# fmfi-compbio/nadavca

Hardware: AMD Instinct MI355X
Metric: reads/sec (align_signal, ~4k-sample reads) (higher is better)
Workload: dtype f64

## Files before the change

### nadavca_amd/csrc/api.hip

```cpp
#include <math.h>
#include <stdarg.h>
#include <stdio.h>
#include <stdlib.h>
#include <string.h>

#include <new>
#include <vector>

#include "nvk_internal.h"

static thread_local char g_err[512] = "";

void nvk_set_error(const char *fmt, ...) {
  va_list ap;
  va_start(ap, fmt);
  vsnprintf(g_err, sizeof g_err, fmt, ap);
  va_end(ap);
}

extern "C" const char *nvk_last_error(void) { return g_err; }

extern "C" int nvk_device_count(void) {
  int n = 0;
  if (hipGetDeviceCount(&n) != hipSuccess) return 0;
// ... 36 lines not shown

int64_t nvk_spill_cap(nvk_ctx *ctx, int which_ws) {
  if (ctx->ws_limit > 0) return ctx->ws_limit;
  const int share = ctx->spill_share > 1 ? ctx->spill_share : 1;
  int64_t cap = ((int64_t)48 << 30) / share;
  size_t free_b = 0, total_b = 0;
  if (hipMemGetInfo(&free_b, &total_b) == hipSuccess)
    cap = (int64_t)((double)(free_b + ctx->ws_bytes[which_ws]) * 0.6 / share);
  const int64_t floor_b = (int64_t)64 << 20;
  return cap > floor_b ? cap : floor_b;
}

TimerScope::TimerScope(nvk_ctx *c, int kid) : ctx(c), id(kid) {
  if (ctx->timing_on) (void)hipEventRecord(ctx->ev0, ctx->stream);
}
TimerScope::~TimerScope() {
  if (ctx->timing_on) {
    (void)hipEventRecord(ctx->ev1, ctx->stream);
    (void)hipEventSynchronize(ctx->ev1);
    float ms = 0.f;
    if (hipEventElapsedTime(&ms, ctx->ev0, ctx->ev1) == hipSuccess) {
      ctx->k_ms[id] += (double)ms;
      ctx->k_launches[id] += 1;
    }
  }
}

extern "C" int nvk_ctx_create(int device, nvk_ctx **out) {
  if (!out) {
    nvk_set_error("nvk_ctx_create: out is NULL");
    return NVK_ERR_INVALID;
  }
  *out = nullptr;
// ... 311 lines not shown
      !anc_off || !out_status) {
    nvk_set_error("negative total or NULL offset/status pointer");
    return NVK_ERR_INVALID;
  }
  NVK_HIP(hipSetDevice(model->ctx->device));
  a = BatchArgs{n_reads, total_signal, total_ref, total_anchors, signal, sig_off, reference, ref_off,
                ctx_before, cb_off, ctx_after, ca_off, anchors, anc_off, bandwidth, mel};
  return NVK_OK;
}

struct PlanHost {
  PlanTotals tot;
  int32_t steps[1];
};

int plan_batch(nvk_model *model, const BatchArgs &a, int mode, PlanTotals &tot, const int **order,
               const int32_t **steps_sorted) {
  nvk_ctx *ctx = model->ctx;
  int64_t n = a.n_reads;
  int64_t rows_total = (mode == PLAN_ALIGN_TRANS) ? 2 * a.total_ref : a.total_ref + n;
  int rc;
  if ((rc = nvk_ws_reserve(ctx, WS_META, (size_t)(n + 1) * sizeof(ReadMeta) + 64))) return rc;
  if ((rc = nvk_ws_reserve(ctx, WS_ROWS, (size_t)(rows_total + 1) * sizeof(RowParam)))) return rc;
  if ((rc = nvk_ws_reserve(ctx, WS_BANDTMP, (size_t)(2 * (a.total_ref + n) + 2) * 8))) return rc;
  if ((rc = nvk_ws_reserve(ctx, WS_MISC, 256))) return rc;
  if ((rc = nvk_ws_reserve(ctx, WS_LANE_F, (size_t)(rows_total + 1) * 48))) return rc;
  if ((rc = nvk_ws_reserve(ctx, WS_LANE_R, (size_t)(rows_total + 1) * 48))) return rc;
  if ((rc = nvk_ws_reserve(ctx, WS_OFFS, (size_t)(rows_total + 1) * sizeof(int32_t)))) return rc;
  if ((rc = nvk_ws_reserve(ctx, WS_STEPS, (size_t)(n + 1) * sizeof(int32_t)))) return rc;
  if ((rc = nvk_grow(&ctx->h_plan, &ctx->h_plan_cap, sizeof(PlanHost) + (size_t)n * sizeof(int32_t), true,
                     "planner results")))
    return rc;
  PlanHost *hp = (PlanHost *)ctx->h_plan;
  PlanTotals *d_tot = nvk_plan_totals(ctx);
  rc = launch_plan(ctx, model->dm, a, mode, (ReadMeta *)ctx->ws[WS_META],
                   (RowParam *)ctx->ws[WS_ROWS], (unsigned long long *)ctx->ws[WS_BANDTMP], d_tot,
                   ctx->ws[WS_LANE_F], ctx->ws[WS_LANE_R], (int32_t *)ctx->ws[WS_OFFS]);
  if (rc) return rc;
  int *ord = nullptr;
  rc = launch_order(ctx, (const ReadMeta *)ctx->ws[WS_META], n, d_tot, &ord, (int32_t *)ctx->ws[WS_STEPS]);
  if (rc) return rc;
  NVK_HIP(hipMemcpyAsync(&hp->tot, d_tot, sizeof(PlanTotals), hipMemcpyDeviceToHost, ctx->stream));
  if (n) NVK_HIP(hipMemcpyAsync(hp->steps, ctx->ws[WS_STEPS], (size_t)n * sizeof(int32_t), hipMemcpyDeviceToHost,
                                ctx->stream));
  NVK_HIP(hipStreamSynchronize(ctx->stream));
  tot = hp->tot;
  *order = ord;
  *steps_sorted = hp->steps;
  ctx->last_cells = (int64_t)tot.cells;
  ctx->last_steps = (int64_t)tot.steps;
  return NVK_OK;
}

}

extern "C" int nvk_expected_signal_batch_dev(nvk_model *model, int64_t n_reads, int64_t total_ref,
                                             const int32_t *reference, const int64_t *ref_off,
                                             const int32_t *ctx_before, const int64_t *cb_off,
                                             const int32_t *ctx_after, const int64_t *ca_off,
                                             double *out) {
  int rc = check_common(model, n_reads, 0, 0);
  if (rc) return rc;
  nvk_ctx *ctx = model->ctx;
  NVK_HIP(hipSetDevice(ctx->device));
  rc = launch_expected(ctx, model->dm, n_reads, total_ref, reference, ref_off, ctx_before, cb_off,
// ... 42 lines not shown
    const int32_t *ctx_after, const int64_t *ca_off, const int32_t *anchors,
    const int64_t *anc_off, int bandwidth, int min_event_length, int model_transitions,
    int32_t *out_events, int32_t *out_status) {
  BatchArgs a;
  int rc = dev_batch(model, n_reads, total_signal, total_ref, total_anchors, signal, sig_off, reference, ref_off,
                     ctx_before, cb_off, ctx_after, ca_off, anchors, anc_off, bandwidth, min_event_length,
                     out_status, a);
  if (rc || n_reads == 0) return rc;
  nvk_ctx *ctx = model->ctx;
  PlanTotals tot;
  const char *force = getenv("NADAVCA_ALIGN_KERNEL");
  ctx->last_retries = 0;
  ctx->last_ties = ctx->last_ties_exact = ctx->last_ties_near = ctx->last_ties_ulp = 0;
  const int *order = nullptr;
  const int32_t *steps_sorted = nullptr;
  rc = plan_batch(model, a, model_transitions ? PLAN_ALIGN_TRANS : PLAN_ALIGN_PLAIN, tot, &order, &steps_sorted);
  if (rc) return rc;
  if ((rc = nvk_ws_reserve(ctx, WS_TIES, (size_t)(n_reads + 8) * sizeof(int32_t)))) return rc;
  NVK_HIP(hipMemsetAsync(ctx->ws[WS_TIES], 0, (size_t)(n_reads + 8) * sizeof(int32_t), ctx->stream));
  ctx->ties_n = n_reads;
  ctx->ties_host = nullptr;
  int32_t *d_ties = (int32_t *)ctx->ws[WS_TIES];
  int *d_retry = (int *)(d_ties + n_reads + 4);
  const ReadMeta *metas = (const ReadMeta *)ctx->ws[WS_META];
  const RowParam *rows = (const RowParam *)ctx->ws[WS_ROWS];
  bool exact_all = force && force[0] == '1';
  int32_t tail[5] = {0, 0, 0, 0, 0};
  auto fetch_counts = [&]() -> int {
    int rc2 = launch_count_flags(ctx, d_ties, n_reads, d_ties + n_reads);
    if (rc2) return rc2;
    NVK_HIP(hipMemcpyAsync(tail, d_ties + n_reads, sizeof tail, hipMemcpyDeviceToHost, ctx->stream));
    NVK_HIP(hipStreamSynchronize(ctx->stream));
    return NVK_OK;
  };
  if (!exact_all) {
    rc = launch_align3(ctx, a, model_transitions ? 1 : 0, metas, tot, order, steps_sorted, out_events, out_status,
                       d_retry);
    if (rc) return rc;
    if ((rc = fetch_counts())) return rc;
    ctx->last_retries = tail[4];
    if (tail[4] > 0) {
      rc = launch_align_retry(ctx, a, model_transitions ? 1 : 0, metas, rows, tot, out_events,
                              out_status);
      if (rc) return rc;
      if ((rc = fetch_counts())) return rc;
    }
  } else {
    rc = launch_align(ctx, a, model_transitions ? 1 : 0, metas, rows, tot, out_events, out_status);
    if (rc) return rc;
    if ((rc = fetch_counts())) return rc;
  }
  ctx->last_ties = tail[0];
  ctx->last_ties_exact = tail[1];
  ctx->last_ties_near = tail[2];
  ctx->last_ties_ulp = tail[3];
  return NVK_OK;
}

namespace {
int ell_run(nvk_model *model, const BatchArgs &a, int model_wobbling, double *out_ll, int32_t *out_status,
            const EllHyp &hyp) {
  int rc;
  const int64_t n_reads = a.n_reads, total_ref = a.total_ref;
  nvk_ctx *ctx = model->ctx;
  const int64_t n = n_reads, nrow = total_ref + n;
  if ((rc = nvk_ws_reserve(ctx, WS_META, (size_t)(n + 1) * sizeof(ReadMeta) + 64))) return rc;
  if ((rc = nvk_ws_reserve(ctx, WS_ROWS, (size_t)(total_ref + 1) * sizeof(FusedParam)))) return rc;
  if ((rc = nvk_ws_reserve(ctx, WS_ROWS2, (size_t)(total_ref + 1) * sizeof(FusedParam)))) return rc;
  if ((rc = nvk_ws_reserve(ctx, WS_BP, (size_t)(3 * nrow + 16) * sizeof(int32_t)))) return rc;
  if ((rc = nvk_ws_reserve(ctx, WS_BANDTMP, (size_t)(2 * nrow + 2) * 8))) return rc;
  if ((rc = nvk_ws_reserve(ctx, WS_MISC, 256))) return rc;
  EllPlan pl;
  pl.metas = (ReadMeta *)ctx->ws[WS_META];
  pl.fwd = (FusedParam *)ctx->ws[WS_ROWS];
  pl.rev = (FusedParam *)ctx->ws[WS_ROWS2];
  pl.bs = (int32_t *)ctx->ws[WS_BP];
  pl.be = pl.bs + nrow;
  pl.rowoff = pl.be + nrow;
  PlanTotals *d_tot = nvk_plan_totals(ctx);
  rc = launch_plan_ell(ctx, model->dm, a, model_wobbling ? 1 : 0, pl,
                       (unsigned long long *)ctx->ws[WS_BANDTMP], d_tot);
// ... 135 lines not shown
```

### nadavca_amd/csrc/kernels_align3.hip

```cpp
#include <math.h>

#include <new>
#include <vector>

#include "nvk_internal.h"
#include "xmath.h"
#include "dens.h"
#include "lane3.h"
#include "wave.h"

namespace {

using dens::density;
using dens::density_begin;
using dens::density_end;
using dens::DensHalf;
using dens::ETN;

constexpr int CH = 64;
static_assert(CH == 64, "a refill is one sample per lane");
constexpr int PF = 8;
constexpr int RU = 16;
constexpr int FT = 16;
static_assert(FT % PF == 0 && 32 % FT == 0, "forward trip");
static_assert(32 % PF == 0 && PF % 2 == 0 && 32 % RU == 0 && RU % 2 == 0, "the step count is a multiple of 32 (kernels_plan.hip)");
constexpr int GBIG = 1 << 24;
constexpr int DMAX = 1000;
constexpr int TARGET = 250;
#define HUGE_V 0x1.0p+900
#define MASS_TOL 1e-9
#define TIE_FLAG_REL (1.0 / (double)(1ull << NVK_TIE_BITS))

typedef int v4i_t __attribute__((ext_vector_type(4)));
__device__ __forceinline__ void spill_store2(__amdgpu_buffer_rsrc_t rs, int lane16, int pair, double v_even,
                                             double v_odd) {
  __builtin_amdgcn_raw_buffer_store_b128(__builtin_bit_cast(v4i_t, make_double2(v_even, v_odd)), rs, lane16,
                                         pair * 1024, 0);
}
__device__ __forceinline__ double2 spill_load2(__amdgpu_buffer_rsrc_t rs, int lane16, int pair) {
  return __builtin_bit_cast(double2, __builtin_amdgcn_raw_buffer_load_b128(rs, lane16, pair * 1024, 0));
}

#define STEP_SYNC()                                                              \
  do {                                                                           \
    if (W == 1) WAVE_SYNC();                                                     \
    else asm volatile("s_waitcnt lgkmcnt(0)\n\ts_barrier" ::: "memory");         \
  } while (0)
#define RING_SYNC()                 \
  do {                              \
    if (W == 1) __syncthreads();    \
    else WAVE_SYNC();               \
  } while (0)

struct Align3Args {
  const ReadMeta *metas;
// ... 779 lines not shown
}

bool select_sweeps(int mel, bool pair, int W, int rsh, Align3Kernel k[2]) {
  switch (mel) {
    case 0: return sweeps_of<0>(pair, W, rsh, k);
    case 1: return sweeps_of<1>(pair, W, rsh, k);
    case 2: return sweeps_of<2>(pair, W, rsh, k);
    case 3: return sweeps_of<3>(pair, W, rsh, k);
    case 4: return sweeps_of<4>(pair, W, rsh, k);
    default: return false;
  }
}

}

int launch_align3(nvk_ctx *ctx, const BatchArgs &a, int transitions, const ReadMeta *metas, const PlanTotals &tot,
                  const int *order, const int32_t *steps_sorted, int32_t *out_events, int32_t *out_status,
                  int *d_retry) {
  static_assert(WS_OFFS < (int)(sizeof(ctx->ws) / sizeof(ctx->ws[0])), "workspace table too small");
  if (a.n_reads == 0) return NVK_OK;
  const int mel = a.mel;
  if (mel < 0 || mel > 4) {
    nvk_set_error("min_event_length %d outside the compiled range 0..4", mel);
    return NVK_ERR_UNSUPPORTED;
  }
  const int max_c = tot.max_c < 1 ? 1 : tot.max_c;
  int rc = nvk_ws_reserve(ctx, WS_MISC, 256);
  if (rc) return rc;
  constexpr int N_COUNTERS = 16;
  static_assert(N_COUNTERS % 2 == 0, "a chunk's reverse / forward pair of counters must not straddle a re-zero");
  int *counter = (int *)ctx->ws[WS_MISC];
  int launches = 0;
  NVK_HIP(hipMemsetAsync(d_retry, 0, sizeof(int), ctx->stream));

  constexpr int C_HARD = 24;
  static_assert(ALIGN1_C_CAP + 4 < 8 && C_HARD + 4 < 32, "no kernel for the rescale period these skews need");
  struct Cls { int hi; int W; };
  Cls cls[2];
  int ncls = 0;
  const int64_t n_wide = (int64_t)tot.n_wide;
  const int max_cw = tot.max_cw < 1 ? 1 : tot.max_cw;
  if (a.n_reads - n_wide > 0 || max_c <= ALIGN1_C_CAP)
    cls[ncls++] = Cls{max_c < ALIGN1_C_CAP ? max_c : ALIGN1_C_CAP, 1};
  if (max_c > ALIGN1_C_CAP) cls[ncls++] = Cls{max_cw < C_HARD ? max_cw : C_HARD, ALIGN3_TEAM_W};
  rc = nvk_ws_reserve(ctx, WS_RSTATE, (size_t)a.n_reads * sizeof(int2));
  if (rc) return rc;
  TimerScope ts_align(ctx, NVK_K_ALIGN);
  for (int k = 0; k < ncls; k++) {
    int c = cls[k].hi;
    const int W = cls[k].W, TLk = 64 * W;
    auto lds_need = [&](int cc, int slot_bytes) {
      const int Hc = (cc + mel > 0 ? cc + mel : 1) + (W > 1 ? 1 : 0);
      int SRc = 256;
      while (SRc < 64 * cc + CH) SRc <<= 1;
      return (size_t)ETN * 8 + (size_t)W * SRc * 8 + (size_t)Hc * TLk * slot_bytes + slot_bytes + 16 + 12 * W;
    };
    while (c > 1 && lds_need(c, 20) > 160 * 1024) --c;
    int rsh = transitions ? 4 : 3;
    while ((1 << rsh) <= c + mel) rsh++;
    Align3Kernel kern[2];
    if (!select_sweeps(mel, transitions != 0, W, rsh, kern)) {
// ... 4 lines not shown
    const int H = (c + mel > 0 ? c + mel : 1) + (W > 1 ? 1 : 0);
    int SR = 256;
    while (SR < 64 * c + CH) SR <<= 1;
    const size_t lds = lds_need(c, 20);
    const size_t lds_rev = lds_need(c, 8);
    if (lds > 160 * 1024) return NVK_ERR_UNSUPPORTED;
    int per_cu = (int)((160 * 1024) / lds);
    if (per_cu > 4 * LB / W) per_cu = 4 * LB / W;
    if (per_cu < 1) per_cu = 1;
    int per_cu_rev = (int)((160 * 1024) / lds_rev);
    if (per_cu_rev > 4 * (W > 1 ? LB_REV_TEAM : LB_REV) / W) per_cu_rev = 4 * (W > 1 ? LB_REV_TEAM : LB_REV) / W;
    if (per_cu_rev < 1) per_cu_rev = 1;
    int32_t mxpad = 1;
    for (int64_t q = 0; q < a.n_reads; q++) mxpad = steps_sorted[q] > mxpad ? steps_sorted[q] : mxpad;
    const int64_t bp_stride = (int64_t)((mxpad + 31) / 32 + 1) * TLk;
    const int64_t cap = nvk_spill_cap(ctx, WS_SPILL);

    Align3Args g;
    g.metas = metas;
    g.fwdl = (const Lane3 *)ctx->ws[WS_LANE_F];
    g.revl = (const Lane3 *)ctx->ws[WS_LANE_R];
    g.offs = (const int32_t *)ctx->ws[WS_OFFS];
    g.signal = a.signal;
    g.bp_stride = bp_stride;
    g.order = order;
    g.H = H;
    g.SR = SR;
    g.transitions = transitions;
    g.c_cap = c;
    g.flag_above = (k == ncls - 1) ? 1 : 0;
    g.rstate = (int2 *)ctx->ws[WS_RSTATE];
// ... 30 lines not shown
      rc = nvk_ws_reserve(ctx, WS_STAGE, (size_t)n_chunk * L_stride * 4);
      if (rc) return rc;
      int64_t slots_f = ctx->slots_override > 0 ? ctx->slots_override : (int64_t)ctx->num_cus * per_cu;
      int64_t slots_r = ctx->slots_override > 0 ? ctx->slots_override : (int64_t)ctx->num_cus * per_cu_rev;
      if (slots_f > n_chunk) slots_f = n_chunk;
      if (slots_r > n_chunk) slots_r = n_chunk;
      rc = nvk_ws_reserve(ctx, WS_BP, (size_t)slots_f * bp_stride * 4);
      if (rc) return rc;
      g.spill_v = (double *)ctx->ws[WS_SPILL];
      g.spill_L = (int32_t *)ctx->ws[WS_STAGE];
      g.bp = (uint32_t *)ctx->ws[WS_BP];
      g.spill_stride = spill_stride;
      g.L_stride = L_stride;
      g.n_reads = (int)n_chunk;
      g.read_lo = (int)lo;
      if (launches % N_COUNTERS == 0) NVK_HIP(hipMemsetAsync(counter, 0, N_COUNTERS * sizeof(int), ctx->stream));
      g.counter = counter + launches % N_COUNTERS;
      hipLaunchKernelGGL(kern[0], dim3((unsigned)slots_r), dim3(TLk), lds_rev, ctx->stream, g);
      g.counter = counter + (launches + 1) % N_COUNTERS;
      hipLaunchKernelGGL(kern[1], dim3((unsigned)slots_f), dim3(TLk), lds, ctx->stream, g);
      launches += 2;
      NVK_HIP(hipGetLastError());
      lo = hi;
    }
  }
  ctx->last_spill_bytes = (int64_t)tot.steps * 64 * 16 + (int64_t)tot.steps / 16 * 8 + (int64_t)tot.steps * 8 * 2;
  return NVK_OK;
}
```

### nadavca_amd/csrc/kernels_plan.hip

```cpp
#include <math.h>

#include "nvk_internal.h"
#include "kmer.h"
#include "lane3.h"
#include "wave.h"

namespace {

__device__ __forceinline__ int read_is_bad(const DeviceModel &dm, const BatchArgs &a, int rd, int tid,
                                           int nthreads) {
  const int64_t s0 = a.sig_off[rd], s1 = a.sig_off[rd + 1], r0 = a.ref_off[rd], r1 = a.ref_off[rd + 1];
  const int64_t a0 = a.anc_off[rd], a1 = a.anc_off[rd + 1];
  const int64_t b0 = a.cb_off[rd], b1 = a.cb_off[rd + 1], c0 = a.ca_off[rd], c1 = a.ca_off[rd + 1];
  const int64_t N64 = s1 - s0, R64 = r1 - r0;
  if (s0 < 0 || r0 < 0 || a0 < 0 || b0 < 0 || c0 < 0 || a1 < a0 || b1 < b0 || c1 < c0 ||
      s1 > a.total_signal || r1 > a.total_ref || a1 > a.total_anchors || b1 - b0 > 0x3fffffff ||
      c1 - c0 > 0x3fffffff)
    return 1;
  if (R64 < 1 || N64 < 1 || N64 > 0x3fffffff || R64 > 0x1fffffff) return 1;
  const int R = (int)R64, A = (int)(a1 - a0), nb = (int)(b1 - b0), na = (int)(c1 - c0);
  const int32_t *anc = a.anchors + 2 * a0;
  const int32_t *ref = a.reference + r0, *cb = a.ctx_before + b0, *ca = a.ctx_after + c0;
  int bad = 0;
  for (int j = tid; j < A && !bad; j += nthreads) {
// ... 119 lines not shown
        unsigned long long w = tbe[j];
        v = (w >> 32) ? (int)(unsigned int)(w & 0xffffffffu) - 1 : N;
      } else {
        v = 0x7fffffff;
      }
      v = min(wave_scan_min_dpp(v), carry);
      carry = __builtin_amdgcn_readlane(v, 63);
      if (j <= R) be[j] = v;
    }
  }
  __syncthreads();
}

__device__ __forceinline__ void plan_rows_lds(const DeviceModel &dm, const PlanRead &q, int mode, double log_p_in,
                                              int c_cap, int rd, ReadMeta m, ReadMeta *metas, RowParam *rows,
                                              Lane3 *lane_f, Lane3 *lane_r, int32_t *lane_offs, PlanShared &sh) {
  const int tid = threadIdx.x, lane = tid & 63, wv = tid >> 6;
  const int32_t *ref = q.ref, *cb = q.cb, *ca = q.ca;
  const int N = q.N, R = q.R, T = q.T, nb = q.nb, na = q.na, mel = q.mel;
  const bool trans = (mode == PLAN_ALIGN_TRANS);
  constexpr int VT = PLAN_VT;
  int *sh_x = (int *)sh.pool, *sh_S = sh_x + VT;
  int *sh_bs = sh_S + VT, *sh_be = sh_bs + PLAN_BCAP;
  plan_bands_lds(q.anc, q.A, R, N, q.bw, sh.pool, sh.pool + PLAN_BCAP, sh_bs, sh_be, tid);

  auto rmel = [=](int r) { return (r + 1 < T && !(trans && (r & 1))) ? mel : 0; };
  auto BS = [=](int r) { return sh_bs[trans ? (r + 1) >> 1 : r]; };
  auto BE = [=](int r) { return sh_be[trans ? (r + 1) >> 1 : r]; };
  auto LO = [=](int r) {
    int lo = BS(r);
    if (r > 0) {
// ... 181 lines not shown
    }
    RowParam p, nx;
    p.mean = __shfl_up(o.mean, 1, 64);
    p.ac = __shfl_up(o.ac, 1, 64);
    p.mc = __shfl_up(o.mc, 1, 64);
    p.bs = p.be = p.lo = p.hi = p.mel = p.off = 0;
    nx.mean = nx.ac = nx.mc = 0.0;
    nx.bs = nx.be = nx.lo = nx.hi = nx.mel = nx.off = 0;
    if (have && lane > 0) {
      o.bs = BS(r);
      o.be = BE(r);
      o.lo = LO(r);
      o.hi = HI(r);
      o.off = OFF(r);
      if (!trans && r > 0 && r + 1 < T) plateau |= (p.mean == o.mean) ? 1 : 0;
      rp[r] = o;
      if (records) {
        if (r > 0) {
          p.bs = BS(r - 1);
          p.be = BE(r - 1);
          p.mel = rmel(r - 1);
          p.off = OFF(r - 1);
        }
        if (r < top) {
          nx.bs = BS(r + 1);
          nx.be = BE(r + 1);
          nx.off = OFF(r + 1);
        }
        const int adv_f = (r >= ST) ? o.off - OFF(r - ST) : 0;
        const int adv_b = (r + ST <= top) ? OFF(r + ST) - o.off : 0;
        Lane3 f, b;
// ... 211 lines not shown
    m.cw = cw;
    m.t_min = t_min;
    m.n_steps = t_max - t_min + 1;
    m.pad = rp[T - 1].hi + off_top - t_min + 1;
    m.pad = (m.pad + 31) & ~31;
    m.cells = cells;
    m.rsv = plateau ? 1 : 0;
    if (badband) m.status = NVK_READ_BAD_BAND;
    metas[rd] = m;
  }
}

__global__ __launch_bounds__(PLAN_T, 5) void plan_kernel(DeviceModel dm, BatchArgs a, int mode,
                                                  double log_p_in, int c_cap, ReadMeta *metas,
                                                  RowParam *rows, unsigned long long *bandtmp,
                                                  Lane3 *lane_f, Lane3 *lane_r, int32_t *lane_offs) {
  const int rd = blockIdx.x;
  const int tid = threadIdx.x;
  __shared__ PlanShared sh;
  if (rd >= a.n_reads) return;
  if (tid == 0) {
    sh.cells = 0ull;
    sh.c = 1;
  }
  const int64_t s0 = a.sig_off[rd], r0 = a.ref_off[rd], a0 = a.anc_off[rd];
  const int64_t N64 = a.sig_off[rd + 1] - s0;
  const int64_t R64 = a.ref_off[rd + 1] - r0;
  const int64_t A64 = a.anc_off[rd + 1] - a0;
  PlanRead q;
  q.nb = (int)(a.cb_off[rd + 1] - a.cb_off[rd]);
  q.na = (int)(a.ca_off[rd + 1] - a.ca_off[rd]);
// ... 26 lines not shown
    m.row_off = r0 + rd;
  }
  m.T = q.T;
  m.c = 1;
  m.t_min = 0;
  m.n_steps = 0;

  int bad = read_is_bad(dm, a, rd, tid, PLAN_T);
  bad = __syncthreads_or(bad);
  if (bad) {
    m.status = NVK_READ_BAD_INPUT;
    if (tid == 0) metas[rd] = m;
    return;
  }
  if (q.R + 1 <= PLAN_BCAP && dm.n <= 0x100000000ll)
    plan_rows_lds(dm, q, mode, log_p_in, c_cap, rd, m, metas, rows, lane_f, lane_r, lane_offs, sh);
  else
    plan_rows_global(dm, q, mode, log_p_in, c_cap, rd, m, metas, rows, bandtmp, lane_f, lane_r, lane_offs, sh);
}

__global__ __launch_bounds__(256) void plan_totals_kernel(const ReadMeta *metas, int n, int c_cap, PlanTotals *totals) {
  const int rd = blockIdx.x * 256 + threadIdx.x, lane = threadIdx.x & 63, wv = threadIdx.x >> 6;
  int steps = 0, c = 0, cw = 0, T = 0, wide = 0;
  unsigned long long cells = 0ull, pad = 0ull;
  if (rd < n) {
    const ReadMeta m = metas[rd];
    if (m.status == NVK_READ_OK) {
      steps = max(m.n_steps, 0), c = max(m.c, 0), cw = max(m.cw, 0), T = max(m.T, 0);
      wide = (m.c > c_cap) ? 1 : 0;
      cells = (unsigned long long)m.cells;
      pad = (unsigned long long)m.pad;
// ... 161 lines not shown
  int pos = (int)(g - ref_off[rd]);
  const int32_t *ref = reference + ref_off[rd], *cb = cbs + cb_off[rd], *ca = cas + ca_off[rd];
  const int64_t id = kmer_id_checked(dm, ref, R, cb, nb, ca, na, pos);
  out[g] = id >= 0 ? dm.mean[id] : (double)NAN;
}


constexpr int ORD_B = 64;
constexpr int ORD_N = 2 * ORD_B;
__device__ __forceinline__ int order_bucket(const ReadMeta &m, int max_steps) {
  if (m.status != NVK_READ_OK) return ORD_N - 1;
  long long b = (long long)m.n_steps * ORD_B / ((long long)max_steps + 1);
  const int sb = ORD_B - 1 - (int)(b < 0 ? 0 : (b > ORD_B - 1 ? ORD_B - 1 : b));
  return (m.cw != 0 ? 0 : ORD_B) + sb;
}
__global__ void order_count_kernel(const ReadMeta *metas, int n, const PlanTotals *tot, int *cnt) {
  int rd = blockIdx.x * blockDim.x + threadIdx.x;
  if (rd < n) atomicAdd(&cnt[order_bucket(metas[rd], tot->max_steps)], 1);
}
__global__ void order_scan_kernel(int *cnt) {
  int lane = threadIdx.x;
  const int v0 = cnt[2 * lane], v1 = cnt[2 * lane + 1], s = wave_scan_add(v0 + v1, lane);
  cnt[2 * lane] = s - v0 - v1;
  cnt[2 * lane + 1] = s - v1;
  cnt[ORD_N + 2 * lane] = 0;
  cnt[ORD_N + 2 * lane + 1] = 0;
}
__global__ void order_fill_kernel(const ReadMeta *metas, int n, const PlanTotals *tot, int *cnt, int *order,
                                  int32_t *steps_out) {
  int rd = blockIdx.x * blockDim.x + threadIdx.x;
  if (rd < n) {
    const ReadMeta m = metas[rd];
    int b = order_bucket(m, tot->max_steps);
    const int pos = cnt[b] + atomicAdd(&cnt[ORD_N + b], 1);
    order[pos] = rd;
    if (steps_out) steps_out[pos] = (m.status == NVK_READ_OK) ? m.pad : 0;
  }
}

__global__ void count_flags_kernel(const int32_t *flags, int64_t n, int32_t *out) {
  int64_t g = (int64_t)blockIdx.x * blockDim.x + threadIdx.x;
  const int f = (g < n) ? flags[g] : 0;
  int v = ((f & 7) != 0) ? 1 : 0, v0 = f & 1, v1 = (f >> 1) & 1, v2 = (f >> 2) & 1;
  v = wave_sum(v), v0 = wave_sum(v0), v1 = wave_sum(v1), v2 = wave_sum(v2);
  if ((threadIdx.x & 63) == 0 && v) {
    atomicAdd(out, v);
    if (v0) atomicAdd(out + 1, v0);
    if (v1) atomicAdd(out + 2, v1);
    if (v2) atomicAdd(out + 3, v2);
// ... 21 lines not shown
  int *cnt = ord + n_reads;
  NVK_HIP(hipMemsetAsync(cnt, 0, 2 * ORD_N * sizeof(int), ctx->stream));
  const unsigned blocks = (unsigned)((n_reads + 255) / 256);
  TimerScope ts(ctx, NVK_K_PLAN);
  hipLaunchKernelGGL(order_count_kernel, dim3(blocks), dim3(256), 0, ctx->stream, metas, (int)n_reads, tot_dev, cnt);
  hipLaunchKernelGGL(order_scan_kernel, dim3(1), dim3(64), 0, ctx->stream, cnt);
  hipLaunchKernelGGL(order_fill_kernel, dim3(blocks), dim3(256), 0, ctx->stream, metas, (int)n_reads, tot_dev, cnt, ord,
                     steps_out);
  NVK_HIP(hipGetLastError());
  *order = ord;
  return NVK_OK;
}

int launch_plan(nvk_ctx *ctx, const DeviceModel &dm, const BatchArgs &a, int mode,
                ReadMeta *metas, RowParam *rows, unsigned long long *bandtmp, PlanTotals *totals,
                void *lane_f, void *lane_r, int32_t *lane_offs) {
  NVK_HIP(hipMemsetAsync(totals, 0, sizeof(PlanTotals), ctx->stream));
  if (a.n_reads == 0) return NVK_OK;
  {
    TimerScope ts(ctx, NVK_K_PLAN);
    const double log_p_in = log(0.01);
    hipLaunchKernelGGL(plan_kernel, dim3((unsigned)a.n_reads), dim3(PLAN_T), 0, ctx->stream, dm, a, mode,
                       log_p_in, ALIGN1_C_CAP, metas, rows, bandtmp, (Lane3 *)lane_f, (Lane3 *)lane_r, lane_offs);
    hipLaunchKernelGGL(plan_totals_kernel, dim3((unsigned)((a.n_reads + 255) / 256)), dim3(256), 0, ctx->stream,
                       metas, (int)a.n_reads, ALIGN1_C_CAP, totals);
  }
  NVK_HIP(hipGetLastError());
  return NVK_OK;
}

int launch_plan_ell(nvk_ctx *ctx, const DeviceModel &dm, const BatchArgs &a, int wobbling,
                    const EllPlan &pl, unsigned long long *bandtmp, PlanTotals *totals) {
  NVK_HIP(hipMemsetAsync(totals, 0, sizeof(PlanTotals), ctx->stream));
  if (a.n_reads == 0) return NVK_OK;
  {
    TimerScope ts(ctx, NVK_K_PLAN);
    hipLaunchKernelGGL(plan_ell_kernel, dim3((unsigned)a.n_reads), dim3(64), 0, ctx->stream, dm, a,
                       wobbling, pl, bandtmp, totals);
  }
  NVK_HIP(hipGetLastError());
  return NVK_OK;
}

// ... 14 lines not shown
```

### nadavca_amd/csrc/nvk_internal.h

```cpp
#pragma once
#include <hip/hip_runtime.h>
#include <stdint.h>

#include <vector>

#include "../../include/nadavca_hip.h"

struct __attribute__((aligned(16))) RowParam {
  double mean, ac, mc;
  int32_t bs, be;
  int32_t lo, hi;
  int32_t mel;
  int32_t off;
};
static_assert(sizeof(RowParam) == 48, "RowParam layout");

struct __attribute__((aligned(16))) FusedParam {
  double b_mean, b_ac, b_mc;
  int32_t wbs, wbe;
  int32_t ebs, ebe;
  int32_t has_wob;
  int32_t store_off;
};
static_assert(sizeof(FusedParam) == 48, "FusedParam layout");
// ... 38 lines not shown

struct nvk_ctx {
  int device;
  hipStream_t stream;
  hipStream_t stream2;
  hipEvent_t ev_fork, ev_join;
  int slots_override;
  int num_cus;
  void *ws[WS_COUNT];
  size_t ws_bytes[WS_COUNT];
  int timing_on;
  double k_ms[NVK_K_COUNT];
  int64_t k_launches[NVK_K_COUNT];
  hipEvent_t ev0, ev1;
  int64_t last_cells, last_steps, last_spill_bytes;
  int64_t last_retries;
  int64_t last_ties;
  int64_t last_ties_exact, last_ties_near, last_ties_ulp;
  int64_t ties_n;
  const int32_t *ties_host;
  int64_t ws_limit;
  void *h_plan;
  size_t h_plan_cap;
  int spill_share;
  struct nvk_pipe_state *pipe;
};

struct nvk_model {
  nvk_ctx *ctx;
  DeviceModel dm;
  double *d_mean, *d_ac, *d_mc;
};


void nvk_set_error(const char *fmt, ...);
void nvk_pipe_release(nvk_ctx *ctx);
void nvk_pipe_set_ws_limit(nvk_ctx *ctx, int64_t bytes);

int nvk_alloc(void **p, size_t bytes, bool pinned, const char *what);
int nvk_grow(void **p, size_t *cap, size_t bytes, bool pinned, const char *what);
int nvk_ws_reserve(nvk_ctx *ctx, int which, size_t bytes);

struct TimerScope {
  nvk_ctx *ctx;
  int id;
  TimerScope(nvk_ctx *c, int kid);
  ~TimerScope();
};

#define NVK_HIP(call)                                                                  \
  do {                                                                                 \
    hipError_t _e = (call);                                                            \
    if (_e != hipSuccess) {                                                            \
      nvk_set_error("%s failed: %s (%s:%d)", #call, hipGetErrorString(_e), __FILE__,   \
                    __LINE__);                                                         \
      return NVK_ERR_HIP;                                                              \
    }                                                                                  \
  } while (0)

struct NvkTmp {
  void *p = nullptr;
// ... 48 lines not shown
  const int32_t *reference;
  const int64_t *ref_off;
  const int32_t *ctx_before;
  const int64_t *cb_off;
  const int32_t *ctx_after;
  const int64_t *ca_off;
  const int32_t *anchors;
  const int64_t *anc_off;
  int bandwidth, mel;
};

enum { PLAN_ALIGN_TRANS = 0, PLAN_ALIGN_PLAIN = 1 };

int launch_plan(nvk_ctx *ctx, const DeviceModel &dm, const BatchArgs &a, int mode,
                ReadMeta *metas, RowParam *rows, unsigned long long *bandtmp, PlanTotals *totals,
                void *lane_f, void *lane_r, int32_t *lane_offs);
int launch_order(nvk_ctx *ctx, const ReadMeta *metas, int64_t n_reads, const PlanTotals *tot_dev, int **order,
                 int32_t *steps_out);
int launch_align(nvk_ctx *ctx, const BatchArgs &a, int transitions, const ReadMeta *metas,
                 const RowParam *rows, const PlanTotals &tot, int32_t *out_events,
                 int32_t *out_status);
struct EllPlan {
  ReadMeta *metas;
  FusedParam *fwd;
  FusedParam *rev;
  int32_t *bs, *be;
  int32_t *rowoff;
};
int launch_plan_ell(nvk_ctx *ctx, const DeviceModel &dm, const BatchArgs &a, int wobbling,
                    const EllPlan &pl, unsigned long long *bandtmp, PlanTotals *totals);
enum class EllKind { Full, Listed, Joint, Edit };
// ... 5 lines not shown
  int64_t total_hyp = 0;
  struct { const int32_t *pos, *base; } listed = {};
  struct { const int64_t *sub_off; const int32_t *sub_pos, *sub_base; } joint = {};
  struct { const int32_t *pos, *del; const int64_t *ins_off; const int32_t *ins_base; } edit = {};
};
int launch_ell(nvk_ctx *ctx, const DeviceModel &dm, const BatchArgs &a, int wobbling,
               const EllPlan &pl, const PlanTotals &tot, double *out_ll, int32_t *out_status, const EllHyp &hyp);
int launch_count_flags(nvk_ctx *ctx, const int32_t *flags, int64_t n, int32_t *out_count);
int64_t nvk_spill_cap(nvk_ctx *ctx, int which_ws);
constexpr int NVK_READ_RETRY_INTERNAL = 2;
constexpr int ALIGN3_TEAM_W = 4;
constexpr int ALIGN1_C_CAP = 3;
int launch_align_retry(nvk_ctx *ctx, const BatchArgs &a, int transitions, const ReadMeta *metas,
                       const RowParam *rows, const PlanTotals &tot, int32_t *out_events,
                       int32_t *out_status);
int launch_align3(nvk_ctx *ctx, const BatchArgs &a, int transitions, const ReadMeta *metas, const PlanTotals &tot,
                  const int *order, const int32_t *steps_sorted, int32_t *out_events, int32_t *out_status,
                  int *d_retry);
int launch_expected(nvk_ctx *ctx, const DeviceModel &dm, int64_t n_reads, int64_t total_ref,
                    const int32_t *reference, const int64_t *ref_off, const int32_t *cb,
                    const int64_t *cb_off, const int32_t *ca, const int64_t *ca_off, double *out);
```

Measured before the change: 672,300.

## Skip row-parameter writes in planning and overlap host prep with plan kernel

The plan kernel now writes the per-row RowParam table only when the exact aligner will need it. On the default align3 path that table is rebuilt lazily, and only if some reads need a retry. Host-side setup (ties memset, counter zeroing, the spill-cap query that calls hipMemGetInfo) moves into a callback that runs while the plan kernel is in flight. The order count/fill kernels now aggregate into shared-memory buckets before touching global atomics, and spill buffer accesses gain a cache-policy aux bit. The costs are an extra plan launch whenever retries occur, and the removal of the d_retry memset, which now relies on the ties memset covering that slot.

```diff
diff --git a/nadavca_amd/csrc/api.hip b/nadavca_amd/csrc/api.hip
--- a/nadavca_amd/csrc/api.hip
+++ b/nadavca_amd/csrc/api.hip
@@ -74,9 +74,13 @@
 TimerScope::TimerScope(nvk_ctx *c, int kid) : ctx(c), id(kid) {
   if (ctx->timing_on) (void)hipEventRecord(ctx->ev0, ctx->stream);
 }
+void TimerScope::stop() {
+  if (ctx->timing_on && !stopped) (void)hipEventRecord(ctx->ev1, ctx->stream);
+  stopped = true;
+}
 TimerScope::~TimerScope() {
   if (ctx->timing_on) {
-    (void)hipEventRecord(ctx->ev1, ctx->stream);
+    if (!stopped) (void)hipEventRecord(ctx->ev1, ctx->stream);
     (void)hipEventSynchronize(ctx->ev1);
     float ms = 0.f;
     if (hipEventElapsedTime(&ms, ctx->ev0, ctx->ev1) == hipSuccess) {
@@ -418,12 +422,13 @@
   int32_t steps[1];
 };
 
-int plan_batch(nvk_model *model, const BatchArgs &a, int mode, PlanTotals &tot, const int **order,
-               const int32_t **steps_sorted) {
+int plan_batch_queue(nvk_model *model, const BatchArgs &a, int mode, int write_rows, const int **order,
+                     const std::function<int()> *meanwhile) {
   nvk_ctx *ctx = model->ctx;
   int64_t n = a.n_reads;
   int64_t rows_total = (mode == PLAN_ALIGN_TRANS) ? 2 * a.total_ref : a.total_ref + n;
   int rc;
+  ctx->rows_current = 0;
   if ((rc = nvk_ws_reserve(ctx, WS_META, (size_t)(n + 1) * sizeof(ReadMeta) + 64))) return rc;
   if ((rc = nvk_ws_reserve(ctx, WS_ROWS, (size_t)(rows_total + 1) * sizeof(RowParam)))) return rc;
   if ((rc = nvk_ws_reserve(ctx, WS_BANDTMP, (size_t)(2 * (a.total_ref + n) + 2) * 8))) return rc;
@@ -432,27 +437,43 @@
   if ((rc = nvk_ws_reserve(ctx, WS_LANE_R, (size_t)(rows_total + 1) * 48))) return rc;
   if ((rc = nvk_ws_reserve(ctx, WS_OFFS, (size_t)(rows_total + 1) * sizeof(int32_t)))) return rc;
   if ((rc = nvk_ws_reserve(ctx, WS_STEPS, (size_t)(n + 1) * sizeof(int32_t)))) return rc;
+  if ((rc = nvk_ws_reserve(ctx, WS_ORDER, (size_t)n * sizeof(int) + 4096))) return rc;
   if ((rc = nvk_grow(&ctx->h_plan, &ctx->h_plan_cap, sizeof(PlanHost) + (size_t)n * sizeof(int32_t), true,
                      "planner results")))
     return rc;
-  PlanHost *hp = (PlanHost *)ctx->h_plan;
   PlanTotals *d_tot = nvk_plan_totals(ctx);
   rc = launch_plan(ctx, model->dm, a, mode, (ReadMeta *)ctx->ws[WS_META],
                    (RowParam *)ctx->ws[WS_ROWS], (unsigned long long *)ctx->ws[WS_BANDTMP], d_tot,
-                   ctx->ws[WS_LANE_F], ctx->ws[WS_LANE_R], (int32_t *)ctx->ws[WS_OFFS]);
-  if (rc) return rc;
+                   ctx->ws[WS_LANE_F], ctx->ws[WS_LANE_R], (int32_t *)ctx->ws[WS_OFFS], write_rows, meanwhile);
+  if (rc) return rc;
+  ctx->rows_current = write_rows ? 1 : 0;
   int *ord = nullptr;
   rc = launch_order(ctx, (const ReadMeta *)ctx->ws[WS_META], n, d_tot, &ord, (int32_t *)ctx->ws[WS_STEPS]);
   if (rc) return rc;
-  NVK_HIP(hipMemcpyAsync(&hp->tot, d_tot, sizeof(PlanTotals), hipMemcpyDeviceToHost, ctx->stream));
+  *order = ord;
+  return NVK_OK;
+}
+
+int plan_batch_wait(nvk_ctx *ctx, int64_t n, PlanTotals &tot, const int32_t **steps_sorted) {
+  PlanHost *hp = (PlanHost *)ctx->h_plan;
+  NVK_HIP(hipMemcpyAsync(&hp->tot, nvk_plan_totals(ctx), sizeof(PlanTotals), hipMemcpyDeviceToHost, ctx->stream));
   if (n) NVK_HIP(hipMemcpyAsync(hp->steps, ctx->ws[WS_STEPS], (size_t)n * sizeof(int32_t), hipMemcpyDeviceToHost,
                                 ctx->stream));
   NVK_HIP(hipStreamSynchronize(ctx->stream));
   tot = hp->tot;
-  *order = ord;
   *steps_sorted = hp->steps;
   ctx->last_cells = (int64_t)tot.cells;
   ctx->last_steps = (int64_t)tot.steps;
+  return NVK_OK;
+}
+
+int plan_rows_now(nvk_model *model, const BatchArgs &a, int mode) {
+  nvk_ctx *ctx = model->ctx;
+  if (ctx->rows_current) return NVK_OK;
+  int rc = launch_plan(ctx, model->dm, a, mode, (ReadMeta *)ctx->ws[WS_META], (RowParam *)ctx->ws[WS_ROWS],
+                       (unsigned long long *)ctx->ws[WS_BANDTMP], nullptr, nullptr, nullptr, nullptr, 1);
+  if (rc) return rc;
+  ctx->rows_current = 1;
   return NVK_OK;
 }
 
@@ -525,17 +546,24 @@
   ctx->last_ties = ctx->last_ties_exact = ctx->last_ties_near = ctx->last_ties_ulp = 0;
   const int *order = nullptr;
   const int32_t *steps_sorted = nullptr;
-  rc = plan_batch(model, a, model_transitions ? PLAN_ALIGN_TRANS : PLAN_ALIGN_PLAIN, tot, &order, &steps_sorted);
-  if (rc) return rc;
+  const bool exact_all = force && force[0] == '1';
+  const int mode = model_transitions ? PLAN_ALIGN_TRANS : PLAN_ALIGN_PLAIN;
   if ((rc = nvk_ws_reserve(ctx, WS_TIES, (size_t)(n_reads + 8) * sizeof(int32_t)))) return rc;
-  NVK_HIP(hipMemsetAsync(ctx->ws[WS_TIES], 0, (size_t)(n_reads + 8) * sizeof(int32_t), ctx->stream));
+  if (!exact_all && (rc = align3_reserve(ctx, n_reads))) return rc;
+  int64_t spill_cap = 0;
+  const std::function<int()> meanwhile = [&]() -> int {
+    NVK_HIP(hipMemsetAsync(ctx->ws[WS_TIES], 0, (size_t)(n_reads + 8) * sizeof(int32_t), ctx->stream));
+    return exact_all ? NVK_OK : align3_prepare(ctx, &spill_cap);
+  };
+  rc = plan_batch_queue(model, a, mode, exact_all ? 1 : 0, &order, &meanwhile);
+  if (rc) return rc;
+  if ((rc = plan_batch_wait(ctx, n_reads, tot, &steps_sorted))) return rc;
   ctx->ties_n = n_reads;
   ctx->ties_host = nullptr;
   int32_t *d_ties = (int32_t *)ctx->ws[WS_TIES];
   int *d_retry = (int *)(d_ties + n_reads + 4);
   const ReadMeta *metas = (const ReadMeta *)ctx->ws[WS_META];
   const RowParam *rows = (const RowParam *)ctx->ws[WS_ROWS];
-  bool exact_all = force && force[0] == '1';
   int32_t tail[5] = {0, 0, 0, 0, 0};
   auto fetch_counts = [&]() -> int {
     int rc2 = launch_count_flags(ctx, d_ties, n_reads, d_ties + n_reads);
@@ -546,17 +574,19 @@
   };
   if (!exact_all) {
     rc = launch_align3(ctx, a, model_transitions ? 1 : 0, metas, tot, order, steps_sorted, out_events, out_status,
-                       d_retry);
+                       d_retry, spill_cap);
     if (rc) return rc;
     if ((rc = fetch_counts())) return rc;
     ctx->last_retries = tail[4];
     if (tail[4] > 0) {
+      if ((rc = plan_rows_now(model, a, mode))) return rc;
       rc = launch_align_retry(ctx, a, model_transitions ? 1 : 0, metas, rows, tot, out_events,
                               out_status);
       if (rc) return rc;
       if ((rc = fetch_counts())) return rc;
     }
   } else {
+    if ((rc = plan_rows_now(model, a, mode))) return rc;
     rc = launch_align(ctx, a, model_transitions ? 1 : 0, metas, rows, tot, out_events, out_status);
     if (rc) return rc;
     if ((rc = fetch_counts())) return rc;
@@ -576,6 +606,7 @@
   nvk_ctx *ctx = model->ctx;
   const int64_t n = n_reads, nrow = total_ref + n;
   if ((rc = nvk_ws_reserve(ctx, WS_META, (size_t)(n + 1) * sizeof(ReadMeta) + 64))) return rc;
+  ctx->rows_current = 0;
   if ((rc = nvk_ws_reserve(ctx, WS_ROWS, (size_t)(total_ref + 1) * sizeof(FusedParam)))) return rc;
   if ((rc = nvk_ws_reserve(ctx, WS_ROWS2, (size_t)(total_ref + 1) * sizeof(FusedParam)))) return rc;
   if ((rc = nvk_ws_reserve(ctx, WS_BP, (size_t)(3 * nrow + 16) * sizeof(int32_t)))) return rc;
diff --git a/nadavca_amd/csrc/kernels_align3.hip b/nadavca_amd/csrc/kernels_align3.hip
--- a/nadavca_amd/csrc/kernels_align3.hip
+++ b/nadavca_amd/csrc/kernels_align3.hip
@@ -31,14 +31,15 @@
 #define MASS_TOL 1e-9
 #define TIE_FLAG_REL (1.0 / (double)(1ull << NVK_TIE_BITS))
 
+constexpr int SPILL_AUX = 2;
 typedef int v4i_t __attribute__((ext_vector_type(4)));
 __device__ __forceinline__ void spill_store2(__amdgpu_buffer_rsrc_t rs, int lane16, int pair, double v_even,
                                              double v_odd) {
   __builtin_amdgcn_raw_buffer_store_b128(__builtin_bit_cast(v4i_t, make_double2(v_even, v_odd)), rs, lane16,
-                                         pair * 1024, 0);
+                                         pair * 1024, SPILL_AUX);
 }
 __device__ __forceinline__ double2 spill_load2(__amdgpu_buffer_rsrc_t rs, int lane16, int pair) {
-  return __builtin_bit_cast(double2, __builtin_amdgcn_raw_buffer_load_b128(rs, lane16, pair * 1024, 0));
+  return __builtin_bit_cast(double2, __builtin_amdgcn_raw_buffer_load_b128(rs, lane16, pair * 1024, SPILL_AUX));
 }
 
 #define STEP_SYNC()                                                              \
@@ -848,9 +849,24 @@
 
 }
 
+constexpr int N_COUNTERS = 16;
+static_assert(N_COUNTERS % 2 == 0, "a chunk's reverse / forward pair of counters must not straddle a re-zero");
+
+int align3_reserve(nvk_ctx *ctx, int64_t n_reads) {
+  int rc = nvk_ws_reserve(ctx, WS_MISC, 256);
+  if (rc) return rc;
+  return nvk_ws_reserve(ctx, WS_RSTATE, (size_t)n_reads * sizeof(int2));
+}
+
+int align3_prepare(nvk_ctx *ctx, int64_t *spill_cap) {
+  NVK_HIP(hipMemsetAsync(ctx->ws[WS_MISC], 0, N_COUNTERS * sizeof(int), ctx->stream));
+  *spill_cap = nvk_spill_cap(ctx, WS_SPILL);
+  return NVK_OK;
+}
+
 int launch_align3(nvk_ctx *ctx, const BatchArgs &a, int transitions, const ReadMeta *metas, const PlanTotals &tot,
                   const int *order, const int32_t *steps_sorted, int32_t *out_events, int32_t *out_status,
-                  int *d_retry) {
+                  int *d_retry, int64_t spill_cap) {
   static_assert(WS_OFFS < (int)(sizeof(ctx->ws) / sizeof(ctx->ws[0])), "workspace table too small");
   if (a.n_reads == 0) return NVK_OK;
   const int mel = a.mel;
@@ -859,13 +875,8 @@
     return NVK_ERR_UNSUPPORTED;
   }
   const int max_c = tot.max_c < 1 ? 1 : tot.max_c;
-  int rc = nvk_ws_reserve(ctx, WS_MISC, 256);
-  if (rc) return rc;
-  constexpr int N_COUNTERS = 16;
-  static_assert(N_COUNTERS % 2 == 0, "a chunk's reverse / forward pair of counters must not straddle a re-zero");
   int *counter = (int *)ctx->ws[WS_MISC];
   int launches = 0;
-  NVK_HIP(hipMemsetAsync(d_retry, 0, sizeof(int), ctx->stream));
 
   constexpr int C_HARD = 24;
   static_assert(ALIGN1_C_CAP + 4 < 8 && C_HARD + 4 < 32, "no kernel for the rescale period these skews need");
@@ -877,8 +888,7 @@
   if (a.n_reads - n_wide > 0 || max_c <= ALIGN1_C_CAP)
     cls[ncls++] = Cls{max_c < ALIGN1_C_CAP ? max_c : ALIGN1_C_CAP, 1};
   if (max_c > ALIGN1_C_CAP) cls[ncls++] = Cls{max_cw < C_HARD ? max_cw : C_HARD, ALIGN3_TEAM_W};
-  rc = nvk_ws_reserve(ctx, WS_RSTATE, (size_t)a.n_reads * sizeof(int2));
-  if (rc) return rc;
+  int rc = NVK_OK;
   TimerScope ts_align(ctx, NVK_K_ALIGN);
   for (int k = 0; k < ncls; k++) {
     int c = cls[k].hi;
@@ -913,7 +923,7 @@
     int32_t mxpad = 1;
     for (int64_t q = 0; q < a.n_reads; q++) mxpad = steps_sorted[q] > mxpad ? steps_sorted[q] : mxpad;
     const int64_t bp_stride = (int64_t)((mxpad + 31) / 32 + 1) * TLk;
-    const int64_t cap = nvk_spill_cap(ctx, WS_SPILL);
+    const int64_t cap = (k == 0) ? spill_cap : nvk_spill_cap(ctx, WS_SPILL);
 
     Align3Args g;
     g.metas = metas;
@@ -974,7 +984,8 @@
       g.L_stride = L_stride;
       g.n_reads = (int)n_chunk;
       g.read_lo = (int)lo;
-      if (launches % N_COUNTERS == 0) NVK_HIP(hipMemsetAsync(counter, 0, N_COUNTERS * sizeof(int), ctx->stream));
+      if (launches > 0 && launches % N_COUNTERS == 0)
+        NVK_HIP(hipMemsetAsync(counter, 0, N_COUNTERS * sizeof(int), ctx->stream));
       g.counter = counter + launches % N_COUNTERS;
       hipLaunchKernelGGL(kern[0], dim3((unsigned)slots_r), dim3(TLk), lds_rev, ctx->stream, g);
       g.counter = counter + (launches + 1) % N_COUNTERS;
diff --git a/nadavca_amd/csrc/kernels_plan.hip b/nadavca_amd/csrc/kernels_plan.hip
--- a/nadavca_amd/csrc/kernels_plan.hip
+++ b/nadavca_amd/csrc/kernels_plan.hip
@@ -157,7 +157,8 @@
 
 __device__ __forceinline__ void plan_rows_lds(const DeviceModel &dm, const PlanRead &q, int mode, double log_p_in,
                                               int c_cap, int rd, ReadMeta m, ReadMeta *metas, RowParam *rows,
-                                              Lane3 *lane_f, Lane3 *lane_r, int32_t *lane_offs, PlanShared &sh) {
+                                              bool write_rows, Lane3 *lane_f, Lane3 *lane_r, int32_t *lane_offs,
+                                              PlanShared &sh) {
   const int tid = threadIdx.x, lane = tid & 63, wv = tid >> 6;
   const int32_t *ref = q.ref, *cb = q.cb, *ca = q.ca;
   const int N = q.N, R = q.R, T = q.T, nb = q.nb, na = q.na, mel = q.mel;
@@ -369,7 +370,7 @@
       o.hi = HI(r);
       o.off = OFF(r);
       if (!trans && r > 0 && r + 1 < T) plateau |= (p.mean == o.mean) ? 1 : 0;
-      rp[r] = o;
+      if (write_rows) rp[r] = o;
       if (records) {
         if (r > 0) {
           p.bs = BS(r - 1);
@@ -611,7 +612,7 @@
 __global__ __launch_bounds__(PLAN_T, 5) void plan_kernel(DeviceModel dm, BatchArgs a, int mode,
                                                   double log_p_in, int c_cap, ReadMeta *metas,
                                                   RowParam *rows, unsigned long long *bandtmp,
-                                                  Lane3 *lane_f, Lane3 *lane_r, int32_t *lane_offs) {
+                                                  Lane3 *lane_f, Lane3 *lane_r, int32_t *lane_offs, int write_rows) {
   const int rd = blockIdx.x;
   const int tid = threadIdx.x;
   __shared__ PlanShared sh;
@@ -668,7 +669,7 @@
     return;
   }
   if (q.R + 1 <= PLAN_BCAP && dm.n <= 0x100000000ll)
-    plan_rows_lds(dm, q, mode, log_p_in, c_cap, rd, m, metas, rows, lane_f, lane_r, lane_offs, sh);
+    plan_rows_lds(dm, q, mode, log_p_in, c_cap, rd, m, metas, rows, write_rows != 0, lane_f, lane_r, lane_offs, sh);
   else
     plan_rows_global(dm, q, mode, log_p_in, c_cap, rd, m, metas, rows, bandtmp, lane_f, lane_r, lane_offs, sh);
 }
@@ -860,9 +861,16 @@
   const int sb = ORD_B - 1 - (int)(b < 0 ? 0 : (b > ORD_B - 1 ? ORD_B - 1 : b));
   return (m.cw != 0 ? 0 : ORD_B) + sb;
 }
-__global__ void order_count_kernel(const ReadMeta *metas, int n, const PlanTotals *tot, int *cnt) {
-  int rd = blockIdx.x * blockDim.x + threadIdx.x;
-  if (rd < n) atomicAdd(&cnt[order_bucket(metas[rd], tot->max_steps)], 1);
+__global__ __launch_bounds__(256) void order_count_kernel(const ReadMeta *metas, int n, const PlanTotals *tot,
+                                                          int *cnt) {
+  __shared__ int lc[ORD_N];
+  for (int b = threadIdx.x; b < ORD_N; b += blockDim.x) lc[b] = 0;
+  __syncthreads();
+  const int rd = blockIdx.x * blockDim.x + threadIdx.x;
+  if (rd < n) atomicAdd(&lc[order_bucket(metas[rd], tot->max_steps)], 1);
+  __syncthreads();
+  for (int b = threadIdx.x; b < ORD_N; b += blockDim.x)
+    if (lc[b]) atomicAdd(&cnt[b], lc[b]);
 }
 __global__ void order_scan_kernel(int *cnt) {
   int lane = threadIdx.x;
@@ -872,13 +880,25 @@
   cnt[ORD_N + 2 * lane] = 0;
   cnt[ORD_N + 2 * lane + 1] = 0;
 }
-__global__ void order_fill_kernel(const ReadMeta *metas, int n, const PlanTotals *tot, int *cnt, int *order,
-                                  int32_t *steps_out) {
-  int rd = blockIdx.x * blockDim.x + threadIdx.x;
+__global__ __launch_bounds__(256) void order_fill_kernel(const ReadMeta *metas, int n, const PlanTotals *tot, int *cnt,
+                                                         int *order, int32_t *steps_out) {
+  __shared__ int lc[ORD_N];
+  for (int b = threadIdx.x; b < ORD_N; b += blockDim.x) lc[b] = 0;
+  __syncthreads();
+  const int rd = blockIdx.x * blockDim.x + threadIdx.x;
+  ReadMeta m;
+  int b = 0, rank = 0;
   if (rd < n) {
-    const ReadMeta m = metas[rd];
-    int b = order_bucket(m, tot->max_steps);
-    const int pos = cnt[b] + atomicAdd(&cnt[ORD_N + b], 1);
+    m = metas[rd];
+    b = order_bucket(m, tot->max_steps);
+    rank = atomicAdd(&lc[b], 1);
+  }
+  __syncthreads();
+  for (int k = threadIdx.x; k < ORD_N; k += blockDim.x)
+    if (lc[k]) lc[k] = cnt[k] + atomicAdd(&cnt[ORD_N + k], lc[k]);
+  __syncthreads();
+  if (rd < n) {
+    const int pos = lc[b] + rank;
     order[pos] = rd;
     if (steps_out) steps_out[pos] = (m.status == NVK_READ_OK) ? m.pad : 0;
   }
@@ -930,19 +950,25 @@
 
 int launch_plan(nvk_ctx *ctx, const DeviceModel &dm, const BatchArgs &a, int mode,
                 ReadMeta *metas, RowParam *rows, unsigned long long *bandtmp, PlanTotals *totals,
-                void *lane_f, void *lane_r, int32_t *lane_offs) {
-  NVK_HIP(hipMemsetAsync(totals, 0, sizeof(PlanTotals), ctx->stream));
-  if (a.n_reads == 0) return NVK_OK;
+                void *lane_f, void *lane_r, int32_t *lane_offs, int write_rows,
+                const std::function<int()> *meanwhile) {
+  if (totals) NVK_HIP(hipMemsetAsync(totals, 0, sizeof(PlanTotals), ctx->stream));
+  if (a.n_reads == 0) return meanwhile ? (*meanwhile)() : NVK_OK;
+  int rc = NVK_OK;
   {
     TimerScope ts(ctx, NVK_K_PLAN);
     const double log_p_in = log(0.01);
     hipLaunchKernelGGL(plan_kernel, dim3((unsigned)a.n_reads), dim3(PLAN_T), 0, ctx->stream, dm, a, mode,
-                       log_p_in, ALIGN1_C_CAP, metas, rows, bandtmp, (Lane3 *)lane_f, (Lane3 *)lane_r, lane_offs);
-    hipLaunchKernelGGL(plan_totals_kernel, dim3((unsigned)((a.n_reads + 255) / 256)), dim3(256), 0, ctx->stream,
-                       metas, (int)a.n_reads, ALIGN1_C_CAP, totals);
+                       log_p_in, ALIGN1_C_CAP, metas, rows, bandtmp, (Lane3 *)lane_f, (Lane3 *)lane_r, lane_offs,
+                       write_rows);
+    if (totals)
+      hipLaunchKernelGGL(plan_totals_kernel, dim3((unsigned)((a.n_reads + 255) / 256)), dim3(256), 0, ctx->stream,
+                         metas, (int)a.n_reads, ALIGN1_C_CAP, totals);
+    ts.stop();
+    if (meanwhile) rc = (*meanwhile)();
   }
   NVK_HIP(hipGetLastError());
-  return NVK_OK;
+  return rc;
 }
 
 int launch_plan_ell(nvk_ctx *ctx, const DeviceModel &dm, const BatchArgs &a, int wobbling,
diff --git a/nadavca_amd/csrc/nvk_internal.h b/nadavca_amd/csrc/nvk_internal.h
--- a/nadavca_amd/csrc/nvk_internal.h
+++ b/nadavca_amd/csrc/nvk_internal.h
@@ -2,6 +2,7 @@
 #include <hip/hip_runtime.h>
 #include <stdint.h>
 
+#include <functional>
 #include <vector>
 
 #include "../../include/nadavca_hip.h"
@@ -76,6 +77,7 @@
   int64_t k_launches[NVK_K_COUNT];
   hipEvent_t ev0, ev1;
   int64_t last_cells, last_steps, last_spill_bytes;
+  int rows_current;
   int64_t last_retries;
   int64_t last_ties;
   int64_t last_ties_exact, last_ties_near, last_ties_ulp;
@@ -106,7 +108,9 @@
 struct TimerScope {
   nvk_ctx *ctx;
   int id;
+  bool stopped = false;
   TimerScope(nvk_ctx *c, int kid);
+  void stop();
   ~TimerScope();
 };
 
@@ -185,7 +189,8 @@
 
 int launch_plan(nvk_ctx *ctx, const DeviceModel &dm, const BatchArgs &a, int mode,
                 ReadMeta *metas, RowParam *rows, unsigned long long *bandtmp, PlanTotals *totals,
-                void *lane_f, void *lane_r, int32_t *lane_offs);
+                void *lane_f, void *lane_r, int32_t *lane_offs, int write_rows,
+                const std::function<int()> *meanwhile = nullptr);
 int launch_order(nvk_ctx *ctx, const ReadMeta *metas, int64_t n_reads, const PlanTotals *tot_dev, int **order,
                  int32_t *steps_out);
 int launch_align(nvk_ctx *ctx, const BatchArgs &a, int transitions, const ReadMeta *metas,
@@ -221,9 +226,11 @@
 int launch_align_retry(nvk_ctx *ctx, const BatchArgs &a, int transitions, const ReadMeta *metas,
                        const RowParam *rows, const PlanTotals &tot, int32_t *out_events,
                        int32_t *out_status);
+int align3_reserve(nvk_ctx *ctx, int64_t n_reads);
+int align3_prepare(nvk_ctx *ctx, int64_t *spill_cap);
 int launch_align3(nvk_ctx *ctx, const BatchArgs &a, int transitions, const ReadMeta *metas, const PlanTotals &tot,
                   const int *order, const int32_t *steps_sorted, int32_t *out_events, int32_t *out_status,
-                  int *d_retry);
+                  int *d_retry, int64_t spill_cap);
 int launch_expected(nvk_ctx *ctx, const DeviceModel &dm, int64_t n_reads, int64_t total_ref,
                     const int32_t *reference, const int64_t *ref_off, const int32_t *cb,
                     const int64_t *cb_off, const int32_t *ca, const int64_t *ca_off, double *out);
```

Measured after the change: 698,400 (median of 6 runs). +3.9%, better.
